# yutiansut/marl-optimal-execution

Hardware: AMD Instinct MI355X
Metric: env-steps/sec (whole node), rmsc03 100-agent market ×4096 envs, 1/2/4/8 GPUs (higher is better)
Workload: dtype int64; 1 GPU; rmsc03 x4096 envs per GPU, full episode per step (config build from seeds + the config's session), seeds 123456789+global_env; envs_per_gpu=4096, global_envs=4096, parallelism=envs sharded, dp1, parity_hash=False, env_errors=0, agents_per_env=64, device=AMD Radeon Graphics, cus=256

## Files before the change

### include/mxa.h

```cpp
#ifndef MXA_H
#define MXA_H
#include <stdint.h>
#ifdef __cplusplus
extern "C" {
#endif

typedef struct mxa_handle mxa_handle;

enum { MXA_RMSC03 = 0, MXA_SPARSE_ZI_100 = 1, MXA_SPARSE_ZI_1000 = 2, MXA_MARKETREPLAY = 3, MXA_RMSC03_RL = 4,
       MXA_VALUE_NOISE = 5 ,
       MXA_RMSC01 = 6 ,
       MXA_RMSC02 = 7 ,
       MXA_OBI_RMSC02 = 8 ,
       MXA_RANDOM_FUND_VALUE = 9 ,
       MXA_RANDOM_FUND_DIVERSE = 10 ,
       MXA_HIST_FUND_VALUE = 11 ,
       MXA_HIST_FUND_DIVERSE = 12 ,
       MXA_MARKETREPLAY_RUNNER = 13 ,
       MXA_MARKETREPLAY_TWAP = 14 ,
       MXA_RMSC03_SBMM = 15, MXA_RMSC03_SBMM_POLL = 16,
       MXA_RMSC03_MM = 17 };
enum {
  MXA_OK = 0, MXA_EINVAL = -1, MXA_EHIP = -2, MXA_ENOMEM = -3, MXA_ERANGE = -4
};
// ... 15 lines not shown
  int64_t last_trade;
  int32_t type, flags;
  int64_t starting_cash;
} mxa_agent_state;

typedef struct {
  int64_t final_fundamental;
  int64_t valuation_int;
  double valuation;
  int32_t kind;
  int32_t err;
} mxa_agent_final;

int mxa_create(int32_t config, int32_t n_envs, const uint32_t* seeds, int32_t device,
               int32_t trace_cap, mxa_handle** out);
int mxa_create_hist(int32_t config, int32_t n_envs, const uint32_t* seeds, int32_t device, int32_t trace_cap,
                    const int64_t* fund_t, const double* fund_v, int32_t n_fund, mxa_handle** out);
typedef struct {
  double mm_pov;
  int32_t mm_min_order_size;
  int32_t mm_window_size;
  int32_t mm_num_ticks;
  int32_t pad;
  int64_t mm_wake_up_freq_ns;
} mxa_mm_params;
mxa_mm_params mxa_mm_defaults(void);
int mxa_create_params(int32_t config, int32_t n_envs, const uint32_t* seeds, const mxa_mm_params* per_env,
                      int32_t device, int32_t trace_cap, mxa_handle** out);
#define MXA_CONFIG_ZI_GROUPS 8
typedef struct {
  int32_t base;
  int32_t log_orders;
  int32_t n_noise, n_value;
  int32_t n_mm, n_momentum;
  int32_t n_zi_groups;
  int32_t zi_q_max;
  int32_t zi_count[MXA_CONFIG_ZI_GROUPS], zi_r_min[MXA_CONFIG_ZI_GROUPS], zi_r_max[MXA_CONFIG_ZI_GROUPS];
  double zi_eta[MXA_CONFIG_ZI_GROUPS];
  double zi_sigma_n, zi_r_bar, zi_kappa, zi_sigma_s, zi_sigma_pv, zi_lambda_a;
  int64_t mkt_open_ns, mkt_close_ns;
  int64_t kernel_start_ns, kernel_stop_ns;
  int64_t noise_wake_open_ns, noise_wake_close_ns;
  int64_t date_ns;
  int64_t starting_cash;
  int64_t default_computation_delay_ns;
  double r_bar, kappa, fund_vol, megashock_lambda_a, megashock_mean, megashock_var;
  double value_sigma_n, value_r_bar, value_kappa, value_sigma_s, value_lambda_a;
  int64_t value_starting_cash;
  mxa_mm_params mm;
  int32_t mom_min_size, mom_max_size;
  int64_t mom_wake_up_freq_ns;
  double lat_low, lat_high;
  int32_t queue_capacity, book_capacity;
} mxa_config;
int mxa_config_defaults(int32_t base, mxa_config* out);
int mxa_config_compile(const mxa_config* cfg, const char* cache_dir, char* path_out, int32_t path_cap);
int mxa_config_key(const mxa_config* cfg, char* out17);
int mxa_config_capacities(const mxa_config* cfg, int32_t out2[2]);
int mxa_create_config(const mxa_config* cfg, int32_t n_envs, const uint32_t* seeds, int32_t device, int32_t trace_cap,
                      const char* cache_dir, mxa_handle** out);
int mxa_config_info(int32_t config, int64_t* out8);
int mxa_set_mm_params(mxa_handle* h, const mxa_mm_params* per_env);
int mxa_resident_envs(const mxa_handle* h);
int mxa_reset(mxa_handle* h, const uint8_t* env_mask);
int mxa_set_id_persistence(mxa_handle* h, int32_t on);
int mxa_launch(mxa_handle* h, int64_t max_pops);
int mxa_sync(mxa_handle* h);
int mxa_run(mxa_handle* h, int64_t chunk, int32_t max_launches, int32_t* launches_out);
int mxa_set_launch_schedule(mxa_handle* h, int64_t first_chunk);
int mxa_set_stop_time(mxa_handle* h, int64_t t_stop_ns);
int mxa_run_until(mxa_handle* h, int64_t t_stop_ns, int64_t* events_out);
int mxa_finalize(mxa_handle* h);
int mxa_read_final(mxa_handle* h, int32_t env, mxa_agent_final* out, int32_t cap);
int mxa_read_summary(mxa_handle* h, mxa_env_summary* out );
int mxa_read_agents(mxa_handle* h, int32_t env, mxa_agent_state* out, int32_t cap);
int mxa_read_book(mxa_handle* h, int32_t env, int32_t side, int64_t* out4, int32_t cap);
int mxa_read_trace(mxa_handle* h, int32_t env, int64_t* out , int64_t cap, int64_t* n);
int mxa_set_seeds(mxa_handle* h, const uint32_t* seeds);
int mxa_write_results(mxa_handle* h, void* device_out);
#define MXA_RECORD_WORDS 12
int mxa_write_records(mxa_handle* h, void* device_out);
#define MXA_COUNTER_WORDS 34
int mxa_read_counters(mxa_handle* h, int64_t* out);
#define MXA_INPLACE_WORDS 4
int mxa_read_inplace(mxa_handle* h, uint64_t* out);
int mxa_read_raw(mxa_handle* h, int32_t env, int64_t offset, int64_t bytes, void* out);
int mxa_layout(const mxa_handle* h, int64_t* offsets8);
int32_t mxa_n_agents(const mxa_handle* h);
int32_t mxa_n_envs(const mxa_handle* h);
int64_t mxa_env_bytes(const mxa_handle* h);
int mxa_set_stream(mxa_handle* h, void* stream);
double mxa_last_kernel_ms(const mxa_handle* h);
const char* mxa_last_error(const mxa_handle* h);
void mxa_destroy(mxa_handle* h);

int mxa_create_replay(const int64_t* t, const int64_t* oid, const int64_t* price, const int64_t* size,
                      const int8_t* buy, int32_t n_rec, int32_t n_envs, int32_t device, int32_t trace_cap,
                      mxa_handle** out);
int mxa_create_replay_runner(const int64_t* t, const int64_t* oid, const int64_t* price, const int64_t* size,
                             const int8_t* buy, int32_t n_rec, int32_t n_envs, int32_t device, int32_t trace_cap,
                             mxa_handle** out);
int mxa_create_replay_twap(const int64_t* t, const int64_t* oid, const int64_t* price, const int64_t* size,
                           const int8_t* buy, int32_t n_rec, int32_t trade, int32_t n_envs, int32_t device,
                           int32_t trace_cap, mxa_handle** out);
int mxa_step(mxa_handle* h, const double* actions, double* obs, int32_t* flags);
int mxa_step_device(mxa_handle* h, const double* d_actions, double* d_obs, int32_t* d_flags);
int mxa_step_many(mxa_handle* h, int32_t k, const double* d_actions, double* d_obs, int32_t* d_flags);
typedef struct mxa_policy {
  const float* params; int32_t n_layers; int32_t dims[9];
  const double* grid0; int32_t n0; const double* grid1; int32_t n1;
  double nh, q0;
  const double* table;
  int32_t test, enough;
  const double* u; const int64_t* rnd;
  const double* eps;
} mxa_policy;
int mxa_step_policy(mxa_handle* h, int32_t k, int32_t first_zero, const mxa_policy* p, double* d_obs,
                    int32_t* d_flags, int64_t* d_a, double* d_act, double* d_state);
int mxa_set_parity_hash(mxa_handle* h, int32_t enabled);
#define MXA_RL_STATE_WORDS 8
int mxa_write_rl_state(mxa_handle* h, double* device_out);
const char* mxa_build_id(void);

typedef struct {
  int64_t t;
  int32_t price;
  int32_t qty;
} mxa_book_rec;
#define MXA_BL_FUNDAMENTAL (-2147483647 - 1)
int mxa_set_book_log(mxa_handle* h, int32_t cap);
#define MXA_BL_EV_RX (-2147483647 - 1 + 256)
#define MXA_BL_EV_NT (MXA_BL_EV_RX + 256)
#define MXA_BL_EV_PLACE (MXA_BL_EV_RX + 512)
#define MXA_BL_EV_END (MXA_BL_EV_RX + 768)
int mxa_set_exchange_log(mxa_handle* h, int32_t on);
int mxa_read_book_log(mxa_handle* h, int32_t env, mxa_book_rec* out, int64_t cap, int64_t* n);

int mxa_rng_probe(int32_t device, uint32_t seed, int32_t mode, double a, double b, int32_t n, double* out);
int mxa_math_probe(int32_t device, int32_t mode, const double* x, const double* y, double* out, int64_t n);
int mxa_policy_probe(void* stream, int32_t n, const float* x, const float* params, int32_t n_layers,
                     const int32_t* dims, int32_t test, int32_t enough, const double* u, const int64_t* rnd,
                     const double* eps, float* q, int64_t* a);

#ifdef __cplusplus
}
#endif
#endif
```

### marl-optimal-execution_amd/csrc/mxa_config.h

```cpp
#pragma once
#include <stddef.h>
#include "mxa_layout.h"
#include "../../include/mxa.h"

namespace mxa_cfg {

constexpr int64_t NS = 1000000000LL;
constexpr int64_t MIN = 60 * NS;
constexpr int64_t HOUR = 60 * MIN;

struct Shape {
  int sq, so;
  bool pl;
  int waves;
  int pw;
  int hot;
  int sql = 0;
};
constexpr int sq_lds(int cfg);
constexpr int lat_lds(int cfg);
constexpr Shape shape(int cfg);
#ifndef MXA_RMSC03_WAVES
#define MXA_RMSC03_WAVES 4
#endif
#ifndef MXA_RMSC01_WAVES
#define MXA_RMSC01_WAVES 4
#endif
#ifndef MXA_W_RMSC02
#define MXA_W_RMSC02 2
#endif
#ifndef MXA_BOOK_LDS_RMSC02
#define MXA_BOOK_LDS_RMSC02 0x34
#endif
#ifndef MXA_PL_RMSC02
#define MXA_PL_RMSC02 1
#endif
#ifndef MXA_SQ_RMSC02
#define MXA_SQ_RMSC02 4
#endif
#ifndef MXA_SO_RMSC02
#define MXA_SO_RMSC02 9
#endif
#ifndef MXA_SQ_Z1K
#define MXA_SQ_Z1K 36
#endif
#ifndef MXA_LAT_LDS_MASK
#define MXA_LAT_LDS_MASK (1 << MXA_CFG_SPARSE_ZI_1000)
#endif
#ifndef MXA_SO_Z1K
#define MXA_SO_Z1K 13
#endif
#ifndef MXA_SO_RFD
#define MXA_SO_RFD 9
#endif
#ifndef MXA_RFD_WAVES
#define MXA_RFD_WAVES 1
#endif
#ifndef MXA_RFD_SQL
#define MXA_RFD_SQL 24
#endif
#ifndef MXA_DIRTY_WB_MASK
#define MXA_DIRTY_WB_MASK ((1 << 9) | (1 << 10) | (1 << 11) | (1 << 12) | (1 << MXA_CFG_RMSC01) | (1 << MXA_CFG_RMSC02))
#endif
#ifndef MXA_SYNC_QUERY_MASK
#define MXA_SYNC_QUERY_MASK ((1 << MXA_CFG_RMSC03) | (1 << MXA_CFG_RMSC03_RL))
#endif
#ifndef MXA_SYNC_VALUE_MASK
#define MXA_SYNC_VALUE_MASK MXA_SYNC_QUERY_MASK
#endif
#ifndef MXA_SYNC_LADDER_MASK
#define MXA_SYNC_LADDER_MASK MXA_SYNC_QUERY_MASK
#endif
#ifndef MXA_LADDER_REPLIES_QUEUED
#define MXA_LADDER_REPLIES_QUEUED 0
#endif
#ifndef MXA_SYNC_BOUND_MASK
#define MXA_SYNC_BOUND_MASK MXA_SYNC_QUERY_MASK
#endif
#ifndef MXA_VALUE_OPEN_EARLY
#define MXA_VALUE_OPEN_EARLY 0
#endif
#ifndef MXA_OPEN_RFD
#define MXA_OPEN_RFD 128
#endif
#ifndef MXA_AUTO_SKIP
#define MXA_AUTO_SKIP 1024
#endif
#ifndef MXA_W_OBI
#define MXA_W_OBI 2
#endif
#ifndef MXA_W_Z1
#define MXA_W_Z1 2
#endif
#ifndef MXA_W_VN
#define MXA_W_VN 2
#endif
#ifndef MXA_RFV_WAVES
#define MXA_RFV_WAVES 2
#endif
#ifndef MXA_RFV_SQL
#define MXA_RFV_SQL 12
#endif
#ifndef MXA_RP_HOT
#define MXA_RP_HOT 2
#endif
constexpr Shape shape_builtin(int cfg) {
  return cfg == MXA_CFG_RMSC03 ? Shape{3, 2, true, MXA_RMSC03_WAVES, 6, 0}
       : cfg == MXA_CFG_RMSC03_SBMM ? Shape{3, 2, true, 4, 8, 0}
       : cfg == MXA_CFG_RMSC03_SBMM_POLL ? Shape{3, 2, true, 4, 6, 0}
       : cfg == MXA_CFG_RMSC03_RL ? Shape{3, 2, true, 4, 8, 0}
       : cfg == MXA_CFG_RMSC03_MM ? Shape{5, 3, true, 3, 6, 0}
       : cfg == MXA_CFG_RMSC01 ? Shape{3, 2, true, MXA_RMSC01_WAVES, 8, 0}
       : cfg == MXA_CFG_RMSC02 ? Shape{MXA_SQ_RMSC02, MXA_SO_RMSC02, MXA_PL_RMSC02 != 0, MXA_W_RMSC02, 8, 0}
       : cfg == MXA_CFG_OBI_RMSC02 ? Shape{4, 3, true, MXA_W_OBI, 8, 0}
       : cfg == MXA_CFG_SPARSE_ZI_100 ? Shape{8, 2, true, MXA_W_Z1, 6, 0}
       : cfg == MXA_CFG_VALUE_NOISE ? Shape{6, 2, true, MXA_W_VN, 6, 0}
       : cfg == MXA_CFG_SPARSE_ZI_1000 ? Shape{MXA_SQ_Z1K, MXA_SO_Z1K, false, 1, 6, 0}
       : (cfg == MXA_CFG_RANDOM_FUND_VALUE || cfg == MXA_CFG_HIST_FUND_VALUE) ? Shape{96, 5, false, MXA_RFV_WAVES, 6, 0, MXA_RFV_SQL}
       : (cfg == MXA_CFG_RANDOM_FUND_DIVERSE || cfg == MXA_CFG_HIST_FUND_DIVERSE)
           ? Shape{96, MXA_SO_RFD, false, MXA_RFD_WAVES, 8, 0, MXA_RFD_SQL}
                                       : Shape{4, 1, true, 2, 8, MXA_RP_HOT};
}
constexpr int sq_lds(int cfg) { return shape(cfg).sql ? shape(cfg).sql : shape(cfg).sq; }
constexpr bool rp_hdr_lds(int cfg) {
  return cfg == MXA_CFG_MARKETREPLAY || cfg == MXA_CFG_MARKETREPLAY_RUNNER || cfg == MXA_CFG_MARKETREPLAY_TWAP;
}
#ifndef MXA_BOOK_LDS_RFV
#define MXA_BOOK_LDS_RFV 0x34
#endif
constexpr int book_lds(int cfg) {
  return cfg == MXA_CFG_RMSC02 ? MXA_BOOK_LDS_RMSC02
         : (cfg >= MXA_CFG_RANDOM_FUND_VALUE && cfg <= MXA_CFG_HIST_FUND_DIVERSE) ? MXA_BOOK_LDS_RFV
                                                                                 : 0;
}
constexpr size_t lds_bytes(int cfg) {
  return (size_t)sq_lds(cfg) * 64 * (12 + (shape(cfg).pl ? 4 * shape(cfg).pw : 0)) + 512
         + (size_t)shape(cfg).hot * 512
         + 1024
         + (size_t)lat_lds(cfg) * 8
         + (rp_hdr_lds(cfg) ? 256 : 0)
         + (size_t)__builtin_popcount(book_lds(cfg)) * shape(cfg).so * 256
         + 256
#ifdef MXA_PROF
         + 1024
#endif
      ;
}

constexpr void base_params(MxaParams& P) {
  P.o_rbar = 1e5;
  P.o_kappa = 1.67e-12;
// ... 705 lines not shown
```

### marl-optimal-execution_amd/csrc/mxa_kernels.hip

```cpp
#pragma once
#include <hip/hip_runtime.h>
#if defined(MXA_ONLY_RMSC03) && !(defined(MXA_ONLY_CFG) && (MXA_ONLY_CFG == 3 || MXA_ONLY_CFG == 4))
#define MXA_NO_GYM
#endif

#ifndef MXA_HINT_MASK
#define MXA_HINT_MASK ((1 << 0) | (1 << 4))
#endif
#ifndef MXA_HINT_GROUPS
#define MXA_HINT_GROUPS 3
#endif
#if defined(MXA_INST_CFG)
#define MXA_HINT_ON (((MXA_HINT_MASK) >> (MXA_INST_CFG)) & 1)
#elif defined(MXA_ONLY_RMSC03) && defined(MXA_ONLY_CFG)
#define MXA_HINT_ON (((MXA_HINT_MASK) >> (MXA_ONLY_CFG)) & 1)
#elif defined(MXA_ONLY_RMSC03)
#define MXA_HINT_ON ((MXA_HINT_MASK) & 1)
#else
#define MXA_HINT_ON 0
#endif
#define MXA_EXPECT_(x, v) __builtin_expect(!!(x), v)
#define MXA_PROB_(x, v, p) __builtin_expect_with_probability(!!(x), v, p)
#if MXA_HINT_ON && ((MXA_HINT_GROUPS) & 1)
#define MXA_LIKELY(x) MXA_EXPECT_(x, 1)
// ... 2495 lines not shown
    if (is_zi) {
      get_spread(1);
      rs(AF_STATE, AS_AWAITING_SPREAD);
    } else {
      rs(AF_STATE, AS_ACTIVE);
    }
  }
  DEV void zi_wakeup() { zi_wakeup_as(true); }
  DEV bool zi_update_estimates(i64& v, int& buy) {
    i64 obs = o_observe(cur, PC.zi_sigma_n);
    i64 q = (i64)((double)rg64(AF_SHARES) / 100);
    if (q >= PC.zi_qmax) buy = 0;
    else if (q <= -PC.zi_qmax) buy = 1;
    else {
      RS A = agent_rs();
      buy = (int)rs_randint(A, 0, 2);
      agent_rs_put(A);
    }
    i64 r_T = bayes_r_T(obs, PC.zi_kappa, PC.zi_rbar, PC.zi_sigma_n, PC.zi_sigma_s);
    q += PC.zi_qmax - 1;
    i64 idx = buy ? q + 1 : q;
    if (idx < 0) idx += 2 * PC.zi_qmax;
    if (idx < 0 || idx >= 2 * PC.zi_qmax) {
      fail(ERR_THETA_INDEX);
      return false;
    }
    v = r_T + (i64)rgi(AF_THETA + (int)idx);
    return true;
  }
  DEV void zi_place() {
    i64 v;
    int buy;
    if (!zi_update_estimates(v, buy)) return;
    int g = rgi(AF_GROUP);
    RS A = agent_rs();
    i64 R = rs_randint(A, PC.zi_rmin[g], (i64)PC.zi_rmax[g] + 1);
    agent_rs_put(A);
    i64 p = buy ? v - R : v + R;
    i32 bid = 0, ask = 0;
    i64 bid_vol = fl(FL_NB) ? (i64)rgi(AF_BIDQ) : 0, ask_vol = fl(FL_NA) ? (i64)rgi(AF_ASKQ) : 0;
    bid = rgi(AF_BID);
    ask = rgi(AF_ASK);
    if (buy && ask_vol > 0) {
      i64 R_ask = v - ask;
      if ((double)R_ask >= PC.zi_eta[g] * (double)R) p = ask;
    } else if (!buy && bid_vol > 0) {
      i64 R_bid = bid - v;
      if ((double)R_bid >= PC.zi_eta[g] * (double)R) p = bid;
    }
    place_limit(100, buy, p);
  }
  DEV void zi_receive(const Msg& m) {
    ta_receive(m, AG_ZI);
    if (rgi(AF_STATE) == AS_AWAITING_SPREAD && m_kind(m) == MK_SPREAD) {
      if (fl(FL_MKT_CLOSED)) return;
      zi_place();
      rs(AF_STATE, AS_AWAITING_WAKEUP);
    }
  }

  DEV void value_wakeup() {
    if (!value_wake_head()) return;
    cancel_all();
    get_spread(1);
    rs(AF_STATE, AS_AWAITING_SPREAD);
  }
  DEV bool value_wake_head() {
    ta_wakeup();
    rs(AF_STATE, AS_INACTIVE);
    if (!fl(FL_HAS_OPEN) || !fl(FL_HAS_CLOSE)) return false;
    fl_set(FL_TRADING, true);
    if (fl(FL_MKT_CLOSED) && fl(FL_DAILY_CLOSE)) return false;
    RS A = agent_rs();
    double dt = rs_exponential(A, 1.0 / PC.v_lambda);
    agent_rs_put(A);
    wakeup_at(cur_agent, cur + py_round(dt));
    if (fl(FL_MKT_CLOSED) && !fl(FL_DAILY_CLOSE)) {
      get_spread(1);
      rs(AF_STATE, AS_AWAITING_SPREAD);
      return false;
    }
    return true;
  }
  DEV void value_place() {
    i64 obs = o_observe(cur, v_sigma_n());
    i64 r_T = bayes_r_T(obs, PC.v_kappa, v_rbar(), v_sigma_n(), PC.v_sigma_s);
    i32 bid, ask;
    bool hb = known_bid(bid), ha = known_ask(ask);
    int buy;
    i64 p;
    RS G = grs(0);
    if (hb && ha) {
      i64 mid = (i64)((double)((i64)ask + bid) / 2);
      i64 spread = (i64)ask - bid;
      if (spread < 0) spread = -spread;
      i64 adj;
      if (rs_double(G) < PC.v_percent_aggr) adj = 0;
      else adj = rs_randint(G, 0, PC.v_depth_spread * spread);
      if (r_T < mid) {
        buy = 0;
        p = bid + adj;
      } else {
        buy = 1;
        p = ask - adj;
      }
    } else {
      buy = (int)rs_randint(G, 0, 2);
      p = r_T;
    }
    grs_put(0, G);
    place_limit(rgi(AF_SIZE), buy, p);
  }
  DEV void value_receive(const Msg& m) {
    ta_receive(m, AG_VALUE);
    if (rgi(AF_STATE) == AS_AWAITING_SPREAD && m_kind(m) == MK_SPREAD) {
      if (fl(FL_MKT_CLOSED)) return;
      value_place();
      rs(AF_STATE, AS_AWAITING_WAKEUP);
    }
  }

  DEV void noise_wakeup() {
    ta_wakeup();
    rs(AF_STATE, AS_INACTIVE);
    if (!fl(FL_HAS_OPEN) || !fl(FL_HAS_CLOSE)) return;
    fl_set(FL_TRADING, true);
    if (fl(FL_MKT_CLOSED) && fl(FL_DAILY_CLOSE)) return;
    i64 wt = rg64(AF_WAKEUP_TIME);
    if (wt > cur) wakeup_at(cur_agent, wt);
    get_spread(1);
    rs(AF_STATE, AS_AWAITING_SPREAD);
  }
  DEV void noise_receive(const Msg& m) {
    ta_receive(m, AG_NOISE);
    if (rgi(AF_STATE) == AS_AWAITING_SPREAD && m_kind(m) == MK_SPREAD) {
      if (fl(FL_MKT_CLOSED)) return;
      RS G = grs(0);
      int buy = (int)rs_randint(G, 0, 2);
      grs_put(0, G);
      i32 bid, ask;
      bool hb = known_bid(bid), ha = known_ask(ask);
      if (buy && ha) place_limit(rgi(AF_SIZE), 1, ask);
      else if (!buy && hb) place_limit(rgi(AF_SIZE), 0, bid);
      rs(AF_STATE, AS_AWAITING_WAKEUP);
    }
  }

  DEV double mm_pov() { if constexpr (PC.mm_rt) return rgd(AF_MM_POV); else return PC.mm_pov; }
  DEV i64 mm_min() { if constexpr (PC.mm_rt) return rgi(AF_MM_MIN); else return PC.mm_min_size; }
  DEV i64 mm_window() { if constexpr (PC.mm_rt) return rgi(AF_MM_WIN); else return PC.mm_window; }
  DEV i64 mm_ticks() { if constexpr (PC.mm_rt) return rgi(AF_MM_TICKS); else return PC.mm_ticks; }
  DEV i64 mm_wake() { if constexpr (PC.mm_rt) return rg64(AF_MM_WAKE); else return PC.mm_wake; }
  DEV void mm_wakeup() {
    if (ta_wakeup()) {
      get_spread(1);
      get_tv(mm_wake());
    }
  }
  DEV void mm_receive(const Msg& m) {
    i64 mid;
    if (mm_note(m, mid)) mm_requote(mid);
  }
  DEV bool mm_note(const Msg& m, i64& mid) {
    ta_receive(m, AG_POVMM);
    mid = rg64(AF_LAST_MID);
    u32 k = m_kind(m);
    if (k == MK_TV && fl(FL_AW_TV)) {
      i64 qty = py_round(mm_pov() * (double)rg64(AF_TV));
      const i64 mn = mm_min();
      if (MXA_UNLIKELY(qty > INT32_MAX)) {
        fail(ERR_ORDER_SIZE);
        return false;
      }
      rs(AF_ORDER_SIZE, (u32)(qty >= mn ? qty : mn));
      fl_set(FL_AW_TV, false);
    }
    if (k == MK_SPREAD && fl(FL_AW_SPREAD)) {
      i32 bid, ask;
      bool hb = known_bid(bid), ha = known_ask(ask);
      if (hb && ha) {
        mid = (i64)((double)((i64)ask + bid) / 2);
        rs64(AF_LAST_MID, mid);
        fl_set(FL_LAST_MID, true);
        fl_set(FL_AW_SPREAD, false);
      }
    }
    return true;
  }
  DEV void mm_requote(i64 mid) {
    if (!fl(FL_AW_SPREAD) && !fl(FL_AW_TV)) {
      cancel_all();
      const i64 ticks = mm_ticks();
      i64 hb = mid - 1, la = mid + mm_window();
      i64 lb = hb - ticks, ha = la + ticks;
      i64 sz = rgi(AF_ORDER_SIZE);
      const int NL = 2 * (int)(ticks + 1);
      if (BATCH && NL <= MM_LADDER_MAX && sz > 0 && rgi(AF_NORD) + NL <= PC.L.open_cap) {
        mm_place_ladder(sz, lb, la, (int)ticks + 1);
      } else {
        for (i64 p = lb; p <= hb; p++) place_limit(sz, 1, p);
        for (i64 p = la; p <= ha; p++) place_limit(sz, 0, p);
      }
// ... 1316 lines not shown
    R->finished = 1;
    if (U(R->rl_trade)) fail(ERR_RP_STOPPING);
  }

  DEV void rl_state_row(double* o) {
    auto R = rh();
    const u64 rec = rec_fetch(PC.first_rl);
    const u32 lo = (u32)rec, hi = (u32)(rec >> 32);
    const i64 cash = (i64)(((u64)rdl(hi, AF_CASH >> 1) << 32) | rdl(lo, AF_CASH >> 1));
    const i64 shares = (i64)(((u64)rdl(hi, AF_SHARES >> 1) << 32) | rdl(lo, AF_SHARES >> 1));
    double v[MXA_RL_STATE_WORDS] = {(double)cash, (double)shares, (double)U(R->rl_exec), 0.0, 0.0, 0.0, 0.0, 0.0};
    if (U(R->m_cnt) > 0) {
      const RpLob l = ring()[U(R->m_head)];
      v[3] = (double)l.bid;
      v[4] = (double)l.ask;
      v[5] = (double)U(R->m_bq);
      v[6] = (double)U(R->m_aq);
      v[7] = (double)(l.flags & 3);
    }
    if (lane == 0)
      for (int i = 0; i < MXA_RL_STATE_WORDS; i++) o[i] = v[i];
  }

  DEV void tw_wakeup() {
    if (!ta_wakeup()) return;
    if (!U(rh()->rl_trade)) return;
    const i32 k = cur < PC.rl_h0 ? 0 : (i32)((cur - PC.rl_h0) / PC.rl_hstep) + 1;
    if (k < PC.rl_nh) wakeup_at(cur_agent, PC.rl_h0 + (i64)k * PC.rl_hstep);
    get_spread(PC.rl_depth);
    rs(AF_STATE, AS_AWAITING_SPREAD);
  }
  DEV void tw_receive(const Msg& m) {
    ta_receive(m, AG_TWAP);
    if (rgi(AF_STATE) != AS_AWAITING_SPREAD || m_kind(m) != MK_SPREAD) return;
    const i64 d = cur - PC.rl_h0;
    if (d < 0 || d % PC.rl_hstep != 0 || d / PC.rl_hstep >= PC.rl_nh) return;
    const i64 k = d / PC.rl_hstep;
    if (k == PC.rl_nh - 2) {
      fail(ERR_TWAP_MARKET);
      return;
    }
    if (k < PC.rl_nh - 2) {
      const u32 f = flags();
      fail((f & FL_NB) && (f & FL_NA) ? ERR_TWAP_SCHEDULE : ERR_TWAP_QUOTE);
    }
  }

  DEV void dispatch(int type, bool wake, const Msg& m) {
    if (wake) {
      if constexpr (PC.n_zi > 0)
        if (type == AG_ZI) return zi_wakeup();
      if constexpr (PC.n_noise > 0)
        if (type == AG_NOISE) return noise_wakeup();
      if constexpr (PC.n_value > 0)
        if (type == AG_VALUE) return value_wakeup();
      if constexpr (PC.n_mm > 0)
        if (type == AG_POVMM) return mm_wakeup();
      if constexpr (PC.n_mom > 0)
        if (type == AG_MOMENTUM) return mom_wakeup();
      if constexpr (PC.n_mk > 0)
        if (type == AG_MKTMAKER) return mk_wakeup();
      if constexpr (PC.n_hbl > 0)
        if (type == AG_HBL) return hbl_wakeup();
      if constexpr (PC.n_obi > 0)
        if (type == AG_OBI) return obi_wakeup();
      if constexpr (PC.n_sb > 0)
        if (type == AG_SBMM) return sb_wakeup();
      if constexpr (RP) {
        if (type == AG_REPLAY) return mr_wakeup();
        if constexpr (TW) {
          if (type == AG_TWAP) return tw_wakeup();
        }
      }
      if constexpr (GYM) {
        if (type == AG_DUMMYRL) return rl_wakeup();
      }
    } else {
      if (type == AG_EXCHANGE) return ex_receive(m);
      if constexpr (PC.n_zi > 0)
        if (type == AG_ZI) return zi_receive(m);
      if constexpr (PC.n_noise > 0)
        if (type == AG_NOISE) return noise_receive(m);
      if constexpr (PC.n_value > 0)
        if (type == AG_VALUE) return value_receive(m);
      if constexpr (PC.n_mm > 0)
        if (type == AG_POVMM) return mm_receive(m);
      if constexpr (PC.n_mom > 0)
        if (type == AG_MOMENTUM) return mom_receive(m);
      if constexpr (PC.n_mk > 0)
        if (type == AG_MKTMAKER) return mk_receive(m);
      if constexpr (PC.n_hbl > 0)
        if (type == AG_HBL) return hbl_receive(m);
      if constexpr (PC.n_obi > 0)
        if (type == AG_OBI) return obi_receive(m);
      if constexpr (PC.n_sb > 0)
        if (type == AG_SBMM) return sb_receive(m);
      if constexpr (RP) {
        if (type == AG_REPLAY) return mr_receive(m);
        if constexpr (TW) {
          if (type == AG_TWAP) return tw_receive(m);
        }
      }
      if constexpr (GYM) {
        if (type == AG_DUMMYRL) return rl_receive(m);
      }
    }
  }

  DEV static i64 round_hundreds(i64 x) {
    i64 q = x / 100, r = x % 100;
    if (r < 0) {
      r += 100;
      q -= 1;
    }
    if (r > 50 || (r == 50 && (q & 1))) q += 1;
    return q;
  }
  DEV void stop(mxa_agent_final* out) {
    for (int a = 1; a < PC.n_agents; a++) {
      rec_load(a);
      const int ty = rgi(AF_TYPE);
      mxa_agent_final f;
      f.final_fundamental = 0;
      f.valuation_int = 0;
      f.valuation = 0.0;
      f.kind = 0;
      f.err = 0;
      const i64 cash = rg64(AF_CASH), start = rg64(AF_START_CASH);
      const i64 H = round_hundreds(rg64(AF_SHARES));
      const u32 fl = flags();
      if (ty == AG_NOISE) {
        f.kind = 2;
        if (!(fl & FL_HAS_KNOWN)) {
          f.err = 1;
        } else if ((fl & FL_NB) && (fl & FL_NA) && rgi(AF_BID) != 0 && rgi(AF_ASK) != 0) {
          const double rT = (double)((i64)rgi(AF_BID) + rgi(AF_ASK)) / 2.0;
          f.valuation = (rT * (double)H + (double)(cash - start)) / (double)start;
        } else if (!(fl & FL_HAS_LAST)) {
          f.err = 1;
        } else if (fl & FL_LAST_FLOAT) {
          f.valuation = ((double)rg64(AF_LAST_TRADE) * (double)H + (double)(cash - start)) / (double)start;
        } else {
          f.valuation = (double)(rg64(AF_LAST_TRADE) * H + cash - start) / (double)start;
        }
      } else if (ty == AG_VALUE || ty == AG_ZI || ty == AG_HBL) {
        const i64 rT = o_observe(rg64(AF_ATIME) - rg64(AF_COMP), 0.0);
        if (MXA_RARE(dirty)) rng_maint();
        f.final_fundamental = rT;
        if (ty == AG_VALUE) {
          f.kind = 2;
          f.valuation = (double)(rT * H + cash - start) / (double)start;
        } else {
          f.kind = 1;
          const int nq = 2 * PC.zi_qmax;
          i64 s = 0;
          if (H > nq - PC.zi_qmax || H < -nq - PC.zi_qmax) {
            f.err = 2;
          } else if (H > 0) {
            for (i64 x = 1; x <= H; x++) s += rgi(AF_THETA + (int)(x + PC.zi_qmax - 1));
          } else if (H < 0) {
            for (i64 x = H + 1; x <= 0; x++) {
              i64 i = x + PC.zi_qmax - 1;
              s -= rgi(AF_THETA + (int)(i < 0 ? i + nq : i));
            }
          }
          f.valuation_int = s + rT * H + cash - start;
        }
// ... 576 lines not shown
      q = msg_make(MK_TV_REQ, cur_agent);
      q.w[1] = (u32)(u64)lookback;
      q.w[2] = (u32)((u64)lookback >> 32);
      account_pop(t, kex, q);
      if (lane == 0) h.kc[MXA_KC_REC] += 2;
    } else {
      pops += 2;
    }
    seq += 4;
    if constexpr (MAXQ_REG) maxq = qcount + 2 > maxq ? qcount + 2 : maxq;
    else if (qcount + 2 > h.max_q) h.max_q = qcount + 2;
    atime_store(0, t);
    i64 mid;
    const Msg rs_ = ex_spread_reply(1, false);
    account_pop(t, kmm, rs_);
    mm_note(rs_, mid);
    const Msg rv = ex_tv_reply(vol, false);
    account_pop(t, kmm, rv);
    if (mm_note(rv, mid)) {
      if constexpr (SYNCL) return 4 + mm_ladder_cycle(t, mid, budget);
      else mm_requote(mid);
    }
    return 4;
  }

  static constexpr bool SYNCV = SYNCQ_BASE && ((((MXA_SYNC_VALUE_MASK)) >> CFG) & 1) && PC.n_value > 0;
  DEV int value_cycle(i64 t, i64 budget) {
    OpenOrder o;
    o.oid = -1;
    o.is_buy = o.qty = o.price = 0;
    if constexpr (MXA_VALUE_OPEN_EARLY != 0) {
      const i32 u0 = rgi(AF_NUSED);
      if (lane < u0 && u0 <= 64) o = open_ptr(cur_agent)[lane];
    }
    if (!value_wake_head()) return 0;
    const i32 u = rgi(AF_NUSED), k = rgi(AF_NORD);
    if constexpr (MXA_VALUE_OPEN_EARLY == 0) {
      if (lane < u && u <= 64) o = open_ptr(cur_agent)[lane];
    }
    const u64 live = bal(o.oid != -1);
    const bool ok = status == ST_RUNNING && cur_agent < ACK_LIMIT && t <= PC.mkt_close && t <= stop_t && k <= 1 && u <= 64 &&
                    __popcll(live) == k && budget >= 3 + 2 * k && qcount + k + 1 <= QCAP &&
                    none_before(t);
    if (MXA_UNLIKELY(!ok)) {
      cancel_all();
      get_spread(1);
      rs(AF_STATE, AS_AWAITING_SPREAD);
      return 0;
    }
    PROF_CNT(108);
    note_inplace(1);
    const u64 kex = ((u64)t << KSH) | MT_MESSAGE, kag = kex | ((u64)cur_agent << 2);
    const bool instr = INSTR && (hash_on || trace);
    bool found = false;
    Msg cr;
    int idx = 0;
    if (k) {
      idx = ctz64(live);
      const Msg cm = msg_order(MK_CANCEL, rdli(o.oid, idx), cur_agent, rdli(o.is_buy, idx), rdli(o.qty, idx), rdli(o.price, idx), 0);
      account_pop(t, kex, cm);
      found = cancel_book(cm, cr);
    }
    if (instr) {
      Msg q = msg_make(MK_SPREAD_REQ, cur_agent);
      q.w[1] = 1u;
      account_pop(t, kex, q);
    } else {
      pops++;
    }
    atime_store(0, t);
    const int np = k + 2 + (found ? 1 : 0);
    seq += (u32)np;
    if constexpr (MAXQ_REG) maxq = qcount + k + 1 > maxq ? qcount + k + 1 : maxq;
    else if (qcount + k + 1 > h.max_q) h.max_q = qcount + k + 1;
    if (found) {
      account_pop(t, kag, cr);
      del_open(idx);
    }
    const Msg r = ex_spread_reply(1, false);
    account_pop(t, kag, r);
    if (instr && lane == 0) h.kc[MXA_KC_REC] += found ? 2 : 1;
    rs(AF_STATE, AS_AWAITING_SPREAD);
    if (MXA_RARE(dirty)) rng_maint();
    value_receive(r);
    return np;
  }

  DEV void run(i64 max_pops) {
    if constexpr (BLOG && EXT) {
      if (pops == 0 && h.blog_n == 0 && h.o_pt >= 0) efo_log(h.o_pt, h.o_pv);
    }
    for (i64 n = 0; n < max_pops && status == ST_RUNNING; n++) {
      if constexpr (GYM) {
        if (end_step) break;
      }
      {
        u64 pv = (u64)env;
        u32 plo = (u32)__builtin_amdgcn_readfirstlane((int)(u32)pv);
        u32 phi = (u32)__builtin_amdgcn_readfirstlane((int)(u32)(pv >> 32));
        asm volatile("" : "+s"(plo), "+s"(phi));
        env = (EnvPtr)(GLBP char*)(((u64)phi << 32) | plo);
        asm volatile("" : "+v"(lane));
      }
      PROF_T(t0);
      u64 key;
      u32 eseq;
      int slot = q_peek(key, eseq);
      if (MXA_UNLIKELY(slot < 0 || !(cur <= stop_t))) {
        status = ST_DONE;
        break;
      }
      i64 t = (i64)(key >> KSH);
      int rcp = (int)((key >> 2) & KRCP);
      int type = (int)(key & 3);
      u64 rv_early = 0;
      if constexpr (EARLY_REC) {
        if (rcp != 0) rv_early = rec_fetch(rcp);
      }
      Msg m = pl_read(slot);
      if constexpr (EARLY_REC) asm volatile("" ::"v"(rv_early));
      if constexpr (RUNS) {
        if (type == MT_MESSAGE && (m.w[0] & MF_RUN) && t <= stop_t && eseq >= run_skip) {
          const u32 k = m_kind(m);
          const bool exr = rcp == 0 && (k == MK_CANCEL || k == MK_LIMIT) && !(t > PC.mkt_close) && !BLOG && !MD;
          const bool ackr = rcp > 0 && rcp < ACK_LIMIT && (k == MK_ACCEPTED || k == MK_CANCELLED);
          if (exr || ackr) {
            PROF_ADD(0, t0);
            const int nr = run_event(key, eseq, t, rcp, k, max_pops - n);
            if (nr > 0) {
#ifdef MXA_PROF
              const int kx = rcp == 0 ? (k == MK_CANCEL ? 0 : 1) : (k == MK_ACCEPTED ? 2 : 3);
              PROF_ADD(34 + kx, t0);
              PROF_CNT(38 + kx);
              if (lane == 0) prof[42 + kx] += nr;
#endif
              n += nr - 1;
              continue;
            }
            PROF_ADD(46, t0);
          }
        }
      }
      if constexpr (ACK_FAST || RP_FAST) {
        if (type == MT_MESSAGE && rcp == 0) {
          cur_agent = 0;
          rlo = rhi = 0;
          PROF_ADD(0, t0);
          account_pop(t, key, m);
          PROF_ADD(32, t0);
          q_remove(slot);
          PROF_ADD(33, t0);
          ex_receive(m);
#ifdef MXA_PROF
          {
            const u32 kk = m_kind(m);
            const int eb = kk == MK_SPREAD_REQ ? 48 : kk == MK_TV_REQ ? 49 : kk == MK_LIMIT ? 50 : kk == MK_CANCEL ? 51 : 52;
            PROF_ADD(eb, t0);
            PROF_CNT(eb + 8);
          }
#endif
          if (MXA_RARE(dirty)) rng_maint();
          PROF_ADD(30, t0);
          atime_store(0, t);
          PROF_ADD(31, t0);
          continue;
        }
        if (type == MT_MESSAGE && (m_kind(m) == MK_ACCEPTED || m_kind(m) == MK_MODIFIED) && rcp > 0 && rcp < ACK_LIMIT) {
          PROF_ADD(0, t0);
// ... 960 lines not shown
```

### marl-optimal-execution_amd/mxabides/_lib.py

```python
import ctypes
import os

PKG_ROOT = os.path.dirname(os.path.dirname(os.path.abspath(__file__)))
LIB_PATH = os.environ.get("MXA_LIB") or os.path.join(PKG_ROOT, "lib", "libmxa.so")

MXA_RMSC03, MXA_SPARSE_ZI_100, MXA_SPARSE_ZI_1000, MXA_MARKETREPLAY, MXA_RMSC03_RL, MXA_VALUE_NOISE = 0, 1, 2, 3, 4, 5
MXA_RMSC01 = 6
MXA_RMSC02 = 7
MXA_OBI_RMSC02 = 8
MXA_RANDOM_FUND_VALUE = 9
MXA_RANDOM_FUND_DIVERSE = 10
MXA_HIST_FUND_VALUE = 11
MXA_HIST_FUND_DIVERSE = 12
MXA_MARKETREPLAY_RUNNER = 13
MXA_MARKETREPLAY_TWAP = 14
MXA_RMSC03_SBMM = 15
MXA_RMSC03_SBMM_POLL = 16
MXA_RMSC03_MM = 17
CONFIG_IDS = {"rmsc03": MXA_RMSC03, "sparse_zi_100": MXA_SPARSE_ZI_100, "sparse_zi_1000": MXA_SPARSE_ZI_1000,
              "value_noise": MXA_VALUE_NOISE, "rmsc01": MXA_RMSC01, "rmsc02": MXA_RMSC02,
              "obi_rmsc02": MXA_OBI_RMSC02, "random_fund_value": MXA_RANDOM_FUND_VALUE,
              "random_fund_diverse": MXA_RANDOM_FUND_DIVERSE, "hist_fund_value": MXA_HIST_FUND_VALUE,
              "hist_fund_diverse": MXA_HIST_FUND_DIVERSE,
              "marketreplay_runner": MXA_MARKETREPLAY_RUNNER,
# ... 37 lines not shown

class Policy(ctypes.Structure):
    _fields_ = [("params", ctypes.c_void_p), ("n_layers", ctypes.c_int32), ("dims", ctypes.c_int32 * 9),
                ("grid0", ctypes.c_void_p), ("n0", ctypes.c_int32), ("grid1", ctypes.c_void_p), ("n1", ctypes.c_int32),
                ("nh", ctypes.c_double), ("q0", ctypes.c_double), ("table", ctypes.c_void_p),
                ("test", ctypes.c_int32), ("enough", ctypes.c_int32), ("u", ctypes.c_void_p), ("rnd", ctypes.c_void_p),
                ("eps", ctypes.c_void_p)]


class AgentFinal(ctypes.Structure):
    _fields_ = [("final_fundamental", ctypes.c_int64), ("valuation_int", ctypes.c_int64), ("valuation", ctypes.c_double),
                ("kind", ctypes.c_int32), ("err", ctypes.c_int32)]


class MmParams(ctypes.Structure):
    _fields_ = [("mm_pov", ctypes.c_double), ("mm_min_order_size", ctypes.c_int32), ("mm_window_size", ctypes.c_int32),
                ("mm_num_ticks", ctypes.c_int32), ("pad", ctypes.c_int32), ("mm_wake_up_freq_ns", ctypes.c_int64)]


_P, _I32, _I64, _U32, _D, _S = (ctypes.c_void_p, ctypes.c_int32, ctypes.c_int64, ctypes.c_uint32, ctypes.c_double,
                                ctypes.c_char_p)
_OUT, _N32, _N64 = ctypes.POINTER(_P), ctypes.POINTER(_I32), ctypes.POINTER(_I64)
_TAPE = [_P, _P, _P, _P, _P, _I32]
BINDINGS = {
    "mxa_create": ([_I32, _I32, _P, _I32, _I32, _OUT], _I32),
    "mxa_create_hist": ([_I32, _I32, _P, _I32, _I32, _P, _P, _I32, _OUT], _I32),
    "mxa_mm_defaults": ([], MmParams),
    "mxa_create_params": ([_I32, _I32, _P, _P, _I32, _I32, _OUT], _I32),
    "mxa_config_defaults": ([_I32, _P], _I32),
    "mxa_config_compile": ([_P, _S, _P, _I32], _I32),
    "mxa_config_key": ([_P, _P], _I32),
    "mxa_config_capacities": ([_P, _P], _I32),
    "mxa_create_config": ([_P, _I32, _P, _I32, _I32, _S, _OUT], _I32),
    "mxa_config_info": ([_I32, _P], _I32),
    "mxa_set_mm_params": ([_P, _P], _I32),
    "mxa_resident_envs": ([_P], _I32),
    "mxa_reset": ([_P, _P], _I32),
    "mxa_set_id_persistence": ([_P, _I32], _I32),
    "mxa_launch": ([_P, _I64], _I32),
    "mxa_sync": ([_P], _I32),
    "mxa_run": ([_P, _I64, _I32, _N32], _I32),
    "mxa_set_launch_schedule": ([_P, _I64], _I32),
    "mxa_set_stop_time": ([_P, _I64], _I32),
    "mxa_run_until": ([_P, _I64, _P], _I32),
    "mxa_finalize": ([_P], _I32),
    "mxa_read_final": ([_P, _I32, _P, _I32], _I32),
    "mxa_read_summary": ([_P, _P], _I32),
    "mxa_read_agents": ([_P, _I32, _P, _I32], _I32),
    "mxa_read_book": ([_P, _I32, _I32, _P, _I32], _I32),
    "mxa_read_trace": ([_P, _I32, _P, _I64, _N64], _I32),
    "mxa_set_seeds": ([_P, _P], _I32),
    "mxa_write_results": ([_P, _P], _I32),
    "mxa_write_records": ([_P, _P], _I32),
    "mxa_read_counters": ([_P, _P], _I32),
    "mxa_read_inplace": ([_P, _P], _I32),
    "mxa_read_raw": ([_P, _I32, _I64, _I64, _P], _I32),
    "mxa_layout": ([_P, _P], _I32),
    "mxa_n_agents": ([_P], _I32),
    "mxa_n_envs": ([_P], _I32),
    "mxa_env_bytes": ([_P], _I64),
    "mxa_set_stream": ([_P, _P], _I32),
    "mxa_last_kernel_ms": ([_P], _D),
    "mxa_last_error": ([_P], _S),
    "mxa_destroy": ([_P], None),
    "mxa_create_replay": (_TAPE + [_I32, _I32, _I32, _OUT], _I32),
    "mxa_create_replay_runner": (_TAPE + [_I32, _I32, _I32, _OUT], _I32),
    "mxa_create_replay_twap": (_TAPE + [_I32, _I32, _I32, _I32, _OUT], _I32),
    "mxa_step": ([_P, _P, _P, _P], _I32),
    "mxa_step_device": ([_P, _P, _P, _P], _I32),
    "mxa_step_many": ([_P, _I32, _P, _P, _P], _I32),
    "mxa_step_policy": ([_P, _I32, _I32, ctypes.POINTER(Policy), _P, _P, _P, _P, _P], _I32),
    "mxa_set_parity_hash": ([_P, _I32], _I32),
    "mxa_write_rl_state": ([_P, _P], _I32),
    "mxa_build_id": ([], _S),
    "mxa_set_book_log": ([_P, _I32], _I32),
    "mxa_set_exchange_log": ([_P, _I32], _I32),
    "mxa_read_book_log": ([_P, _I32, _P, _I64, _N64], _I32),
    "mxa_rng_probe": ([_I32, _U32, _I32, _D, _D, _I32, _P], _I32),
    "mxa_math_probe": ([_I32, _I32, _P, _P, _P, _I64], _I32),
    "mxa_policy_probe": ([_P, _I32, _P, _P, _I32, _N32, _I32, _I32, _P, _P, _P, _P, _P], _I32),
}
EXPORTS = list(BINDINGS)
COUNTER_WORDS = 34
INPLACE_WORDS = 4
RECORD_WORDS = 12

_lib = None


class MxaError(RuntimeError):
    pass


def load():
    global _lib
    if _lib is not None:
        return _lib
    if not os.path.exists(LIB_PATH):
        raise MxaError("libmxa.so not built (%s); run __graft_entry__.build()" % LIB_PATH)
    L = ctypes.CDLL(LIB_PATH)
    for name, (argtypes, restype) in BINDINGS.items():
        if hasattr(L, name):
            f = getattr(L, name)
            f.argtypes, f.restype = argtypes, restype
    _lib = L
    return L


def build_id():
    L = load()
    return L.mxa_build_id().decode() if hasattr(L, "mxa_build_id") else "unknown"
```

Baseline: 23.80 billion env-steps/s.

## Place value-agent resting limit orders in place during synchronous spread handling

```diff
diff --git a/include/mxa.h b/include/mxa.h
--- a/include/mxa.h
+++ b/include/mxa.h
@@ -121,7 +121,7 @@
 int mxa_write_records(mxa_handle* h, void* device_out);
 #define MXA_COUNTER_WORDS 34
 int mxa_read_counters(mxa_handle* h, int64_t* out);
-#define MXA_INPLACE_WORDS 4
+#define MXA_INPLACE_WORDS 6
 int mxa_read_inplace(mxa_handle* h, uint64_t* out);
 int mxa_read_raw(mxa_handle* h, int32_t env, int64_t offset, int64_t bytes, void* out);
 int mxa_layout(const mxa_handle* h, int64_t* offsets8);
diff --git a/marl-optimal-execution_amd/csrc/mxa_config.h b/marl-optimal-execution_amd/csrc/mxa_config.h
--- a/marl-optimal-execution_amd/csrc/mxa_config.h
+++ b/marl-optimal-execution_amd/csrc/mxa_config.h
@@ -67,6 +67,12 @@
 #endif
 #ifndef MXA_SYNC_VALUE_MASK
 #define MXA_SYNC_VALUE_MASK MXA_SYNC_QUERY_MASK
+#endif
+#ifndef MXA_SYNC_ORDER_MASK
+#define MXA_SYNC_ORDER_MASK MXA_SYNC_QUERY_MASK
+#endif
+#ifndef MXA_ORDER_ACK_QUEUED
+#define MXA_ORDER_ACK_QUEUED 0
 #endif
 #ifndef MXA_SYNC_LADDER_MASK
 #define MXA_SYNC_LADDER_MASK MXA_SYNC_QUERY_MASK
diff --git a/marl-optimal-execution_amd/csrc/mxa_kernels.hip b/marl-optimal-execution_amd/csrc/mxa_kernels.hip
--- a/marl-optimal-execution_amd/csrc/mxa_kernels.hip
+++ b/marl-optimal-execution_amd/csrc/mxa_kernels.hip
@@ -2601,7 +2601,8 @@
     }
     return true;
   }
-  DEV void value_place() {
+  template <bool INPL = false>
+  DEV int value_place(i64 room = 0) {
     i64 obs = o_observe(cur, v_sigma_n());
     i64 r_T = bayes_r_T(obs, PC.v_kappa, v_rbar(), v_sigma_n(), PC.v_sigma_s);
     i32 bid, ask;
@@ -2628,15 +2629,25 @@
       p = r_T;
     }
     grs_put(0, G);
+    if constexpr (INPL) {
+      if (hb && ha) {
+        const i32 pi = (i32)p;
+        return value_order(rgi(AF_SIZE), buy, pi, buy ? pi < ask : pi > bid, room);
+      }
+    }
     place_limit(rgi(AF_SIZE), buy, p);
-  }
-  DEV void value_receive(const Msg& m) {
+    return 0;
+  }
+  template <bool INPL = false>
+  DEV int value_receive(const Msg& m, i64 room = 0) {
     ta_receive(m, AG_VALUE);
+    int n = 0;
     if (rgi(AF_STATE) == AS_AWAITING_SPREAD && m_kind(m) == MK_SPREAD) {
-      if (fl(FL_MKT_CLOSED)) return;
-      value_place();
+      if (fl(FL_MKT_CLOSED)) return 0;
+      n = value_place<INPL>(room);
       rs(AF_STATE, AS_AWAITING_WAKEUP);
     }
+    return n;
   }
 
   DEV void noise_wakeup() {
@@ -4119,7 +4130,7 @@
       if constexpr (PC.n_noise > 0)
         if (type == AG_NOISE) return noise_receive(m);
       if constexpr (PC.n_value > 0)
-        if (type == AG_VALUE) return value_receive(m);
+        if (type == AG_VALUE) return (void)value_receive(m);
       if constexpr (PC.n_mm > 0)
         if (type == AG_POVMM) return mm_receive(m);
       if constexpr (PC.n_mom > 0)
@@ -4862,8 +4873,45 @@
     if (instr && lane == 0) h.kc[MXA_KC_REC] += found ? 2 : 1;
     rs(AF_STATE, AS_AWAITING_SPREAD);
     if (MXA_RARE(dirty)) rng_maint();
+    if constexpr (SYNCO) return np + value_receive<true>(r, budget - 1 - np);
     value_receive(r);
     return np;
+  }
+  static constexpr bool SYNCO = SYNCV && ((((MXA_SYNC_ORDER_MASK)) >> CFG) & 1);
+  static constexpr bool ORDER_AQ = MXA_ORDER_ACK_QUEUED != 0;
+  DEV int value_order(i64 qty, int is_buy, i32 price, bool rests, i64 room) {
+    const i64 oid = next_order_id();
+    const i32 n = rgi(AF_NORD), u = rgi(AF_NUSED);
+    const bool ok = rests && qty > 0 && room >= 2 && h.b_count < SO * 64 && n < PC.L.open_cap && u < PC.L.open_cap &&
+                    status == ST_RUNNING;
+    if (!ok) {
+      place_limit_oid(qty, is_buy, price, oid);
+      return 0;
+    }
+    PROF_CNT(116);
+    note_inplace(4);
+    if (lane == 0) {
+      OpenOrder o;
+      o.oid = (i32)oid;
+      o.is_buy = is_buy;
+      o.qty = (i32)qty;
+      o.price = price;
+      open_ptr(cur_agent)[u] = o;
+    }
+    rs(AF_NUSED, (u32)(u + 1));
+    rs(AF_NORD, (u32)(n + 1));
+    const u64 kag = ((u64)cur << KSH) | ((u64)cur_agent << 2) | MT_MESSAGE;
+    const Msg am = msg_order(MK_ACCEPTED, (i32)oid, cur_agent, is_buy, (i32)qty, price, 0);
+    if (INSTR && (hash_on || trace)) {
+      account_pop(cur, ((u64)cur << KSH) | MT_MESSAGE, msg_order(MK_LIMIT, (i32)oid, cur_agent, is_buy, (i32)qty, price, 0));
+      if constexpr (!ORDER_AQ) account_pop(cur, kag, am);
+    } else {
+      pops += ORDER_AQ ? 1 : 2;
+    }
+    if constexpr (ORDER_AQ) q_push(kag, seq + 1, am);
+    seq += 2;
+    ex_limit_book(lane == 0, is_buy, price, (i32)oid, cur_agent, (i32)qty);
+    return ORDER_AQ ? 1 : 2;
   }
 
   DEV void run(i64 max_pops) {
diff --git a/marl-optimal-execution_amd/mxabides/_lib.py b/marl-optimal-execution_amd/mxabides/_lib.py
--- a/marl-optimal-execution_amd/mxabides/_lib.py
+++ b/marl-optimal-execution_amd/mxabides/_lib.py
@@ -143,7 +143,7 @@
 }
 EXPORTS = list(BINDINGS)
 COUNTER_WORDS = 34
-INPLACE_WORDS = 4
+INPLACE_WORDS = 6
 RECORD_WORDS = 12
 
 _lib = None
```

New measurement: 25.08 billion env-steps/s, median of 6. +5.4%, better.
